# mrafidashti/neuradar

Measured on NVIDIA B200. Metric: train_step_rays_per_sec, higher is better.
Workload: dtype f32

## Files before the change

### neuradar_b200/csrc/field_fused.cu

```cuda
#include <algorithm>
#include <cstdlib>

#include <cuda.h>
#include <cuda_bf16.h>

#include "actor_grid.cuh"
#include "hash_bwd_plan.cuh"
#include "tc_common.cuh"

namespace nrb {

using namespace tc;

struct FusedParams {
  const float* w[5];
  const float* b[5];
  const float* beta;
  float beta_min;
};

__device__ constexpr int kLK[5] = {32, 32, 48, 32, 32};
__device__ constexpr int kLN[5] = {32, 48, 32, 32, 32};
__device__ constexpr int kLOut[5] = {32, 33, 32, 32, 32};

// ... 20 lines not shown
                   smem_u32(dst_smem)),
               "l"(src_gmem), "r"(bytes), "r"(smem_u32(mbar))
               : "memory");
}

__device__ __forceinline__ void mma_bf16_ss(uint32_t d_tmem, uint64_t a_desc, uint64_t b_desc, uint32_t idesc, bool acc) {
  asm volatile(
      "{\n\t"
      ".reg .pred p;\n\t"
      "setp.ne.b32 p, %4, 0;\n\t"
      "tcgen05.mma.cta_group::1.kind::f16 [%0], %1, %2, %3, p;\n\t"
      "}\n" ::"r"(d_tmem),
      "l"(a_desc), "l"(b_desc), "r"(idesc), "r"(static_cast<uint32_t>(acc))
      : "memory");
}

__device__ __forceinline__ void mma_bf16_ts(uint32_t d_tmem, uint32_t a_tmem, uint64_t b_desc, uint32_t idesc, bool acc) {
  asm volatile(
      "{\n\t"
      ".reg .pred p;\n\t"
      "setp.ne.b32 p, %4, 0;\n\t"
      "tcgen05.mma.cta_group::1.kind::f16 [%0], [%1], %2, %3, p;\n\t"
      "}\n" ::"r"(d_tmem),
      "r"(a_tmem), "l"(b_desc), "r"(idesc), "r"(static_cast<uint32_t>(acc))
      : "memory");
}

__device__ __forceinline__ uint32_t idesc_bf16(int m, int n, int a_mn_major, int b_mn_major) {
  return (1u << 4) | (1u << 7) | (1u << 10) | (static_cast<uint32_t>(a_mn_major) << 15) |
         (static_cast<uint32_t>(b_mn_major) << 16) | (static_cast<uint32_t>(n >> 3) << 17) |
         (static_cast<uint32_t>(m >> 4) << 24);
}

constexpr int kFGroups = 3;
constexpr int kFThreads = kFGroups * kRows;
constexpr int kFCols = 144;
constexpr int kFAcc = 0, kFAHi = 48, kFALo = 96;

__host__ __device__ constexpr int ff_w_floats(int l) { return l == 0 ? 32 * 32 : l == 1 ? 48 * 32 : l == 2 ? 32 * 48 : 32 * 32; }
__host__ __device__ constexpr int ff_w_hi(int l) {
  int o = 0;
  for (int i = 0; i < l; ++i) o += 2 * ff_w_floats(i) * 4;
  return o;
}
__host__ __device__ constexpr int ff_w_lo(int l) { return ff_w_hi(l) + ff_w_floats(l) * 4; }

struct FusedFwdSmem {
  static constexpr int bias = ff_w_hi(5);
  static constexpr int bounce = bias + 5 * 48 * 4;
  static constexpr int mbar = bounce + (kFThreads / 32) * 4096;
  static constexpr int tmem = mbar + 8 * kFGroups;
  static constexpr int total = tmem + 16;
};

struct FusedFwdArgs {
  const float* xyz;
  const float* std;
  const float* x;
  const float* sh;
  int samples_per_ray;
  int64_t M;
  float* feature;
  float* sdf;
  float* alpha;
  uint4* ximg;
  uint32_t* masks;
  int64_t ld;
  ActorGridsDev ag;
  ActorSamplesDev as;
};

template <int F, bool kActors>
__global__ void __launch_bounds__(kFThreads, 1) field_fused_fwd_kernel(const __grid_constant__ FusedParams prm,
                                                                       const __grid_constant__ GridDev grid,
                                                                       const __grid_constant__ FusedFwdArgs a) {
  extern __shared__ __align__(128) char smem[];
  const int t = threadIdx.x, lane = t & 31, r = t & (kRows - 1);
  const int uwarp = uniform_warp_idx();
  const int g = uwarp >> 2;
  float* s_bias = reinterpret_cast<float*>(smem + FusedFwdSmem::bias);
  uint64_t* mbar = reinterpret_cast<uint64_t*>(smem + FusedFwdSmem::mbar) + g;
  uint32_t* tmem_slot = reinterpret_cast<uint32_t*>(smem + FusedFwdSmem::tmem);
  char* bounce = smem + FusedFwdSmem::bounce + uwarp * 4096;

  for (int l = 0; l < 5; ++l) {
    stage_weight_split(prm.w[l], kLOut[l], kLN[l], kLK[l], smem + ff_w_hi(l), smem + ff_w_lo(l));
    for (int j = t; j < 48; j += kFThreads) s_bias[l * 48 + j] = (j < kLOut[l] && prm.b[l] != nullptr) ? __ldg(prm.b[l] + j) : 0.0f;
  }
  if (uwarp == 0) tmem_alloc<512>(tmem_slot);
  if (t == 0)
    for (int i = 0; i < kFGroups; ++i) mbar_init(reinterpret_cast<uint64_t*>(smem + FusedFwdSmem::mbar) + i, 1);
  fence_async_smem();
  fence_before_sync();
  __syncthreads();
  fence_after_sync();
  const uint32_t tg = *tmem_slot + static_cast<uint32_t>(g * kFCols);
  const uint32_t lane_base = tg + (static_cast<uint32_t>((uwarp & 3) * 32) << 16);
  const float beta = fabsf(__ldg(prm.beta)) + prm.beta_min;
  const bool train = a.ximg != nullptr;
  uint32_t phase = 0;

  auto run_layer = [&](int l) {
    fence_before_sync();
    group_barrier(g);
    if ((uwarp & 3) == 0) {
      if (elect_one()) {
        fence_after_sync();
        issue_gemm_ts(tg + kFAcc, kLN[l], tg + kFAHi, tg + kFALo, smem_u32(smem + ff_w_hi(l)), smem_u32(smem + ff_w_lo(l)),
                      kLK[l], kLK[l]);
        mma_commit(mbar);
      }
      __syncwarp();
    }
    mbar_wait(mbar, phase);
    phase ^= 1;
    fence_after_sync();
  };

  const int64_t tiles = (a.M + kRows - 1) / kRows;
  for (int64_t tile = blockIdx.x + static_cast<int64_t>(g) * gridDim.x; tile < tiles;
       tile += static_cast<int64_t>(kFGroups) * gridDim.x) {
    const int64_t row = tile * kRows + r;
    const bool ok = row < a.M;
    const int64_t rr = ok ? row : (a.M - 1);
    float v[32];
    int agid = -1;
    if constexpr (kActors) agid = __ldg(a.as.grid_id + rr);
    if (kActors && agid >= 0) {
      float o16[16];
      actor_gather16(a.ag, agid, __ldg(a.as.pos + 3 * rr), __ldg(a.as.pos + 3 * rr + 1), __ldg(a.as.pos + 3 * rr + 2),
                     __ldg(a.as.std + rr), o16);
#pragma unroll
      for (int j = 0; j < 16; ++j) {
        v[j] = o16[j];
        v[16 + j] = 0.0f;
      }
    } else if constexpr (F > 0) {
      const float px = __ldg(a.xyz + 3 * rr), py = __ldg(a.xyz + 3 * rr + 1), pz = __ldg(a.xyz + 3 * rr + 2);
      const float sd = a.std != nullptr ? __ldg(a.std + rr) : 0.0f;
      const uint32_t hmask = (1u << grid.log2_size) - 1u;
      constexpr int kBatch = 8 / F;
#pragma unroll
      for (int l0 = 0; l0 < 32 / F; l0 += kBatch) {
        Cell c[kBatch];
        float f[kBatch][8][F];
#pragma unroll
        for (int i = 0; i < kBatch; ++i) {
          c[i] = locate_cell(px, py, pz, grid.scalings[l0 + i], hmask);
          const float* base = grid.table + (static_cast<size_t>(l0 + i) << grid.log2_size) * F;
#pragma unroll
          for (int k = 0; k < 8; ++k) load_row<F>(base, c[i].row[k], f[i][k]);
        }
#pragma unroll
        for (int i = 0; i < kBatch; ++i) {
          const float ax = c[i].ox, bx = 1.0f - c[i].ox, ay = c[i].oy, by = 1.0f - c[i].oy, az = c[i].oz, bz = 1.0f - c[i].oz;
          const float w = a.std != nullptr ? level_weight(grid.scalings[l0 + i], sd) : 1.0f;
#pragma unroll
          for (int j = 0; j < F; ++j) {
            const float f03 = f[i][0][j] * ax + f[i][3][j] * bx;
            const float f12 = f[i][1][j] * ax + f[i][2][j] * bx;
            const float f56 = f[i][5][j] * ax + f[i][6][j] * bx;
            const float f47 = f[i][4][j] * ax + f[i][7][j] * bx;
            const float f0312 = f03 * ay + f12 * by;
            const float f4756 = f47 * ay + f56 * by;
            v[(l0 + i) * F + j] = (f0312 * az + f4756 * bz) * w;
          }
        }
      }
    } else {
      float4 pf[8];
      warp_load_rows_coalesced(a.x, tile * kRows + (uwarp & 3) * 32, a.M, lane, pf);
      warp_bounce_to_rows(bounce, lane, pf, v);
    }
    tmem_store_row_split<32>(tg, uwarp, kFAHi, kFALo, 0, v);
    if (train) {
#pragma unroll
      for (int q = 0; q < 4; ++q) {
        uint32_t h[4], m[4];
#pragma unroll
        for (int c = 0; c < 4; ++c) split_bf16_pair(v[8 * q + 2 * c], v[8 * q + 2 * c + 1], h[c], m[c]);
        uint4* dst = a.ximg + tile * 1024 + q * 128 + r;
        dst[0] = make_uint4(h[0], h[1], h[2], h[3]);
        dst[512] = make_uint4(m[0], m[1], m[2], m[3]);
      }
    }
    auto relu_mask = [&](const float* bias) {
      uint32_t m = 0;
#pragma unroll
      for (int j = 0; j < 32; ++j) {
        v[j] = fmaxf(v[j] + bias[j], 0.0f);
        m |= (v[j] > 0.0f ? 1u : 0u) << j;
      }
      return m;
    };
    run_layer(0);
    tmem_load_row<32>(tg + kFAcc, uwarp, 0, v);
    const uint32_t m_h1 = relu_mask(s_bias);
    tmem_store_row_split<32>(tg, uwarp, kFAHi, kFALo, 0, v);
    run_layer(1);
    float sdf_v;
    float emb[32];
    {
      float geo[48];
      tmem_load_row<48>(tg + kFAcc, uwarp, 0, geo);
      sdf_v = geo[0] + s_bias[48];
#pragma unroll
      for (int j = 0; j < 32; ++j) emb[j] = geo[1 + j] + s_bias[48 + 1 + j];
    }
    tmem_store_row_split<32>(tg, uwarp, kFAHi, kFALo, 0, emb);
    {
      float shv[16];
      if (kActors && agid >= 0) {
        sh16_of_direction(__ldg(a.as.dirs + 3 * rr), __ldg(a.as.dirs + 3 * rr + 1), __ldg(a.as.dirs + 3 * rr + 2), shv);
      } else {
        const float4* shp = reinterpret_cast<const float4*>(a.sh + (rr / a.samples_per_ray) * 16);
#pragma unroll
        for (int c = 0; c < 4; ++c) {
          const float4 q4 = __ldg(shp + c);
          shv[4 * c] = q4.x;
          shv[4 * c + 1] = q4.y;
          shv[4 * c + 2] = q4.z;
          shv[4 * c + 3] = q4.w;
        }
      }
      tmem_store_row_split<16>(tg, uwarp, kFAHi, kFALo, 32, shv);
    }
    run_layer(2);
    tmem_load_row<32>(tg + kFAcc, uwarp, 0, v);
    const uint32_t m_g1 = relu_mask(s_bias + 2 * 48);
    tmem_store_row_split<32>(tg, uwarp, kFAHi, kFALo, 0, v);
    run_layer(3);
    tmem_load_row<32>(tg + kFAcc, uwarp, 0, v);
    const uint32_t m_g2 = relu_mask(s_bias + 3 * 48);
    tmem_store_row_split<32>(tg, uwarp, kFAHi, kFALo, 0, v);
    if (train && ok) {
      a.masks[row] = m_h1;
      a.masks[a.ld + row] = m_g1;
      a.masks[2 * a.ld + row] = m_g2;
    }
    run_layer(4);
    tmem_load_row<32>(tg + kFAcc, uwarp, 0, v);
#pragma unroll
    for (int j = 0; j < 32; ++j) v[j] = emb[j] + (v[j] + s_bias[4 * 48 + j]);
    warp_store_rows_coalesced(a.feature, tile * kRows + (uwarp & 3) * 32, a.M, bounce, lane, v);
    if (ok) {
      a.sdf[row] = sdf_v;
      a.alpha[row] = 1.0f / (1.0f + expf(sdf_v * beta));
    }
  }
  fence_before_sync();
  __syncthreads();
  if (uwarp == 0) tmem_free<512>(*tmem_slot);
}

constexpr int kBGroups = 2;
constexpr int kBWorkers = kBGroups * kRows;
constexpr int kBIssuers = 1;
constexpr int kBThreads = kBWorkers + kBIssuers * 32;
constexpr int kBCols = 112;
constexpr int kBAcc = 0, kBAHi = 32, kBAMid = 56, kBDHi = 80, kBDMid = 96;
__device__ constexpr int kDwCol[5] = {224, 224, 368, 296, 296};
__device__ constexpr int kDwLane[5] = {0, 16, 0, 0, 16};
constexpr int kSdfCol = 368, kSdfLane = 16;

struct FusedBwdSmem {
  static constexpr int d_hi = 0, d_mid = 8192;
  static constexpr int d_sdf = 16384;
  static constexpr int d_bytes = 18432;
  static constexpr int h1 = d_bytes;
  static constexpr int emb = h1 + 18432;
  static constexpr int g1 = emb + 26624;
  static constexpr int g2x = g1 + 18432;
  static constexpr int group_bytes = g2x + 18432;
  static constexpr int w = kBGroups * group_bytes;
  static constexpr int w_bytes = 4 * 4096 + 6144;
  static constexpr int w1row0 = w + w_bytes;
// ... 562 lines not shown
              "nrb_field_fused_fwd: pass either a grid (+ xyz) to gather from or the hash features x");
  int F = 0;
  GridDev gd{};
  if (grid != nullptr) {
    if (int rc = check_grid(grid)) return rc;
    NRB_REQUIRE(xyz != nullptr, NRB_ERR_BAD_ARG, "nrb_field_fused_fwd: xyz is null");
    F = grid->features_per_level;
    NRB_REQUIRE((F == 2 || F == 4) && grid->num_levels * F == 32, NRB_ERR_UNSUPPORTED,
                "nrb_field_fused_fwd: the fused gather needs num_levels * features_per_level == 32 with 2 or 4 features");
    gd = to_dev(grid);
  } else {
    NRB_REQUIRE(aligned16(x), NRB_ERR_ALIGNMENT, "nrb_field_fused_fwd: x must be 16-byte aligned");
  }
  NRB_REQUIRE(aligned16(sh) && aligned16(feature), NRB_ERR_ALIGNMENT, "nrb_field_fused_fwd: sh and feature must be 16-byte aligned");
  if (M == 0) return NRB_OK;
  FusedFwdArgs a{};
  a.xyz = xyz, a.std = std, a.x = x, a.sh = sh, a.samples_per_ray = samples_per_ray, a.M = M;
  a.feature = feature, a.sdf = sdf, a.alpha = alpha;
  if (saved != nullptr && saved->ximg != nullptr) {
    NRB_REQUIRE(saved->masks != nullptr && saved->ld >= M && saved->ld % tc::kRows == 0 && aligned16(saved->ximg),
                NRB_ERR_BAD_ARG, "nrb_field_fused_fwd: saved.masks / saved.ld (nrb_field_saved_ld(M)) / alignment");
    a.ximg = static_cast<uint4*>(saved->ximg), a.masks = saved->masks, a.ld = saved->ld;
  }
  const bool actors = actor_grids != nullptr;
  if (actors) {
    if (int rc = check_actor_grids("nrb_field_fused_fwd", actor_grids)) return rc;
    NRB_REQUIRE(grid != nullptr && actor_samples && actor_samples->grid_id && actor_samples->pos && actor_samples->std &&
                    actor_samples->dirs,
                NRB_ERR_BAD_ARG, "nrb_field_fused_fwd: actors need the gather mode and all per-sample actor arrays");
    a.ag = to_dev(actor_grids);
    a.as = ActorSamplesDev{actor_samples->grid_id, actor_samples->pos, actor_samples->std, actor_samples->dirs};
  }
  const int64_t tiles = (M + tc::kRows - 1) / tc::kRows;
  const unsigned nblk = static_cast<unsigned>(std::min<int64_t>((tiles + kFGroups - 1) / kFGroups, sm_count()));
  auto s = static_cast<cudaStream_t>(stream);
#define NRB_FUSED_FWD(FF, AA)                                                                                                  \
  {                                                                                                                            \
    cudaError_t e = ensure_dynamic_smem(reinterpret_cast<const void*>(field_fused_fwd_kernel<FF, AA>), FusedFwdSmem::total); \
    NRB_REQUIRE(e == cudaSuccess, static_cast<int>(e), "nrb_field_fused_fwd: cudaFuncSetAttribute: %s", cudaGetErrorString(e));  \
    field_fused_fwd_kernel<FF, AA><<<nblk, kFThreads, FusedFwdSmem::total, s>>>(fused_params(p), gd, a);                       \
  }
  if (F == 2 && actors) NRB_FUSED_FWD(2, true) else if (F == 4 && actors) NRB_FUSED_FWD(4, true)
  else if (F == 2) NRB_FUSED_FWD(2, false) else if (F == 4) NRB_FUSED_FWD(4, false) else NRB_FUSED_FWD(0, false)
#undef NRB_FUSED_FWD
  return finish_launch("nrb_field_fused_fwd");
}

extern "C" int nrb_field_fused_bwd(const nrb_field_mlp_t* p, const nrb_field_fused_bwd_in_t* in,
                                   const nrb_field_fused_bwd_out_t* out, int32_t samples_per_ray, int64_t M,
                                   nrb_stream_t stream) {
  NRB_REQUIRE(p && in && out && M >= 0 && samples_per_ray > 0, NRB_ERR_BAD_ARG, "nrb_field_fused_bwd: null pointer or bad size");
  NRB_REQUIRE(in->saved.ximg && in->saved.masks && in->sh && in->sdf && in->alpha, NRB_ERR_BAD_ARG,
              "nrb_field_fused_bwd: a required input is null");
  NRB_REQUIRE((in->dfeature != nullptr) != (in->dfeat_ray != nullptr && in->weights != nullptr), NRB_ERR_BAD_ARG,
              "nrb_field_fused_bwd: pass either dfeature [M,32] or dfeat_ray [rays,32] with weights [M]");
  NRB_REQUIRE(in->saved.ld >= M && in->saved.ld % tc::kRows == 0, NRB_ERR_BAD_ARG,
              "nrb_field_fused_bwd: saved.ld must be nrb_field_saved_ld(M)");
  for (int l = 0; l < 5; ++l) NRB_REQUIRE(p->weights[l] != nullptr, NRB_ERR_BAD_ARG, "nrb_field_fused_bwd: weights[%d] is null", l);
  NRB_REQUIRE(p->beta != nullptr, NRB_ERR_BAD_ARG, "nrb_field_fused_bwd: beta is null");
  NRB_REQUIRE(aligned16(in->saved.ximg) && aligned16(in->sh) && (in->dfeature == nullptr || aligned16(in->dfeature)) &&
                  (in->dfeat_ray == nullptr || aligned16(in->dfeat_ray)) && (out->dximg == nullptr || aligned16(out->dximg)),
              NRB_ERR_ALIGNMENT, "nrb_field_fused_bwd: arrays must be 16-byte aligned");
  if (M == 0) return NRB_OK;
  FusedBwdArgs a{};
  a.ximg = static_cast<const uint4*>(in->saved.ximg), a.masks = in->saved.masks, a.ld = in->saved.ld;
  a.sh = in->sh, a.sdf = in->sdf, a.alpha = in->alpha;
  a.dfeature = in->dfeature, a.dfeat_ray = in->dfeat_ray, a.weights = in->weights, a.dsdf = in->dsdf, a.dalpha = in->dalpha;
// ... 29 lines not shown
```

### neuradar_b200/csrc/hash_bwd_plan.cuh

```cuda
#pragma once

#include <algorithm>

#include "common.cuh"

namespace nrb {

struct GridDev {
  const float* table;
  float scalings[NRB_MAX_LEVELS];
  int num_levels;
  int log2_size;
};

inline GridDev to_dev(const nrb_grid_t* g) {
  GridDev d;
  d.table = g->table;
  for (int i = 0; i < NRB_MAX_LEVELS; ++i) d.scalings[i] = g->scalings[i];
  d.num_levels = g->num_levels;
  d.log2_size = g->log2_hashmap_size;
  return d;
}

struct BwdPlan {
  float* scratch;
  int64_t offset[NRB_MAX_LEVELS];
  int64_t stride[NRB_MAX_LEVELS];
  int copies[NRB_MAX_LEVELS];
  int r1[NRB_MAX_LEVELS];
};

template <int F>
__device__ __forceinline__ void scatter_row(float* __restrict__ base, uint32_t row, const float (&v)[F]) {
  float* p = base + static_cast<size_t>(row) * F;
  if constexpr (F == 1) {
    atomicAdd(p, v[0]);
  } else if constexpr (F == 2) {
    atomicAdd(reinterpret_cast<float2*>(p), make_float2(v[0], v[1]));
  } else {
    atomicAdd(reinterpret_cast<float4*>(p), make_float4(v[0], v[1], v[2], v[3]));
  }
}

template <int F>
__device__ __forceinline__ void scatter_x_pair(float* __restrict__ base, uint32_t row_f, uint32_t row_c,
                                               const float (&vf)[F], const float (&vc)[F]) {
  if (row_c == row_f) {
    float t[F];
#pragma unroll
    for (int j = 0; j < F; ++j) t[j] = vf[j] + vc[j];
    scatter_row<F>(base, row_f, t);
    return;
  }
  if constexpr (F <= 2) {
    if (row_c == (row_f ^ 1u)) {
      const bool f_low = (row_f & 1u) == 0;
      float* p = base + static_cast<size_t>(row_f & ~1u) * F;
      if constexpr (F == 1) {
        atomicAdd(reinterpret_cast<float2*>(p), f_low ? make_float2(vf[0], vc[0]) : make_float2(vc[0], vf[0]));
      } else {
        atomicAdd(reinterpret_cast<float4*>(p), f_low ? make_float4(vf[0], vf[1], vc[0], vc[1])
                                                      : make_float4(vc[0], vc[1], vf[0], vf[1]));
      }
      return;
    }
  }
  scatter_row<F>(base, row_f, vf);
  scatter_row<F>(base, row_c, vc);
}

template <int F>
__device__ __forceinline__ void scatter_rows8(float* __restrict__ base, const uint32_t (&row)[8], const float (&v)[8][F]) {
  scatter_x_pair<F>(base, row[3], row[0], v[3], v[0]);
  scatter_x_pair<F>(base, row[2], row[1], v[2], v[1]);
  scatter_x_pair<F>(base, row[7], row[4], v[7], v[4]);
  scatter_x_pair<F>(base, row[6], row[5], v[6], v[5]);
}

template <int F>
__device__ __forceinline__ void scatter_corners(const BwdPlan& plan, int l, int log2_size, int xf, int yf, int zf, int xc,
                                                int yc, int zc, const uint32_t (&hashed_rows)[8], const float (&v)[8][F],
                                                float* __restrict__ dtable, unsigned spread) {
  const int copies = plan.copies[l];
  if (copies > 1) {
    const int R1 = plan.r1[l];
    if (xf >= 0 && yf >= 0 && zf >= 0 && xc < R1 && yc < R1 && zc < R1) {
      float* rep = plan.scratch + plan.offset[l] + static_cast<size_t>(spread % static_cast<unsigned>(copies)) * plan.stride[l];
      const int cx[8] = {xc, xc, xf, xf, xc, xc, xf, xf};
      const int cy[8] = {yc, yf, yf, yc, yc, yf, yf, yc};
      const int cz[8] = {zc, zc, zc, zc, zf, zf, zf, zf};
      uint32_t rows[8];
#pragma unroll
      for (int k = 0; k < 8; ++k) rows[k] = static_cast<uint32_t>((cz[k] * R1 + cy[k]) * R1 + cx[k]);
      scatter_rows8<F>(rep, rows, v);
      return;
    }
  }
  scatter_rows8<F>(dtable + (static_cast<size_t>(l) << log2_size) * F, hashed_rows, v);
}

constexpr int kMergeMaxRuns = 26;

template <int F>
__device__ __forceinline__ void merge_runs_and_scatter(const BwdPlan& plan, int l, int log2_size, float px, float py,
                                                       float pz, float scal, const Cell& c, float (&v)[8][F], bool valid,
                                                       int lane, float* __restrict__ dtable, unsigned spread) {
  const float sx = mul(px, scal), sy = mul(py, scal), sz = mul(pz, scal);
  const int xf = static_cast<int>(floorf(sx)), yf = static_cast<int>(floorf(sy)), zf = static_cast<int>(floorf(sz));
  const int xc = static_cast<int>(ceilf(sx)), yc = static_cast<int>(ceilf(sy)), zc = static_cast<int>(ceilf(sz));
  const int ceq = (xc == xf ? 1 : 0) | (yc == yf ? 2 : 0) | (zc == zf ? 4 : 0) | (valid ? 8 : 0);
  const int pxf = __shfl_up_sync(kFull, xf, 1), pyf = __shfl_up_sync(kFull, yf, 1), pzf = __shfl_up_sync(kFull, zf, 1);
  const int pce = __shfl_up_sync(kFull, ceq, 1);
  const bool head = lane == 0 || pxf != xf || pyf != yf || pzf != zf || pce != ceq;
  const unsigned heads = __ballot_sync(kFull, head);
  bool issue = valid;
  if (__popc(heads) <= kMergeMaxRuns) {
    const unsigned above = heads & ~((2u << lane) - 1u);
    const int next_head = above != 0 ? __ffs(above) - 1 : 32;
#pragma unroll
    for (int d = 1; d < 32; d <<= 1) {
      const bool take = lane + d < next_head;
      if (!__any_sync(kFull, take)) break;
#pragma unroll
      for (int k = 0; k < 8; ++k)
#pragma unroll
        for (int j = 0; j < F; ++j) {
          const float t = __shfl_down_sync(kFull, v[k][j], d);
          if (take) v[k][j] += t;
        }
    }
    issue = valid && head;
// ... 53 lines not shown
```

### neuradar_b200/csrc/proposal_fused.cu

```cuda
#include "actor_grid.cuh"
#include "common.cuh"
#include "hash_bwd_plan.cuh"

namespace nrb {

constexpr int kPropWarps = 4;
constexpr int kMaxChunks = NRB_MAX_SAMPLES / 32;

struct PropGrid {
  const float* table;
  float scalings[NRB_MAX_LEVELS];
  const float* decoder;
  int num_levels;
  int log2_size;
  const int32_t* agid;
  const float* apos;
  const float* astd;
  ActorGridsDev ag;
  float* adtables[NRB_MAX_ACTORS];
};

template <int F, bool kSave>
__global__ void __launch_bounds__(kPropWarps * 32) proposal_fwd_kernel(
    const __grid_constant__ PropGrid g, const float* __restrict__ origins, const float* __restrict__ directions,
// ... 49 lines not shown
      } else {
        for (int l = 0; l < g.num_levels; ++l) {
          const float scal = g.scalings[l];
          const Cell c = locate_cell(q.x, q.y, q.z, scal, mask);
          float v[F];
          interpolate<F>(g.table + (static_cast<size_t>(l) << g.log2_size) * F, c, v);
          const float lw = level_weight(scal, q.std);
#pragma unroll
          for (int j = 0; j < F; ++j) {
            const float f = v[j] * lw;
            pre = fmaf(f, s_dec[l * F + j], pre);
            if constexpr (kSave) saved_feats[(n * S + i) * LF + l * F + j] = f;
          }
        }
      }
      dens = expf(pre);
      if constexpr (kSave) saved_pre[n * S + i] = pre;
      if (density != nullptr) density[n * S + i] = dens;
      dd = mul(sub(end, start), dens);
    }
    const float incl = warp_inclusive_sum(dd, lane);
    float excl = __shfl_up_sync(kFull, incl, 1);
    if (lane == 0) excl = 0.0f;
    const float alpha = 1.0f - expf(-dd);
    const float trans = expf(-(carry + excl));
    if (ok) weights[n * S + i] = nan_to_num(alpha * trans);
    carry += __shfl_sync(kFull, incl, 31);
  }
}

template <int F, int kChunks>
__global__ void __launch_bounds__(kPropWarps * 32) proposal_bwd_kernel(
    const __grid_constant__ PropGrid g, const __grid_constant__ BwdPlan plan, const float* __restrict__ origins, const float* __restrict__ directions,
    const float* __restrict__ pixel_area, float scale, nrb_intervals_t iv, int64_t N,
    const float* __restrict__ saved_feats, const float* __restrict__ saved_pre, const float* __restrict__ dweights,
    const float* __restrict__ ddensity, float* __restrict__ dtable, float* __restrict__ ddecoder) {
  __shared__ float s_ddec[NRB_MAX_LEVELS * 4];
  __shared__ float s_dec[NRB_MAX_LEVELS * 4];
  const int lane = threadIdx.x & 31;
  const int S = iv.num_samples;
  const int LF = g.num_levels * F;
  if (threadIdx.x < NRB_MAX_LEVELS * 4) {
    s_ddec[threadIdx.x] = 0.0f;
    s_dec[threadIdx.x] = threadIdx.x < LF ? g.decoder[threadIdx.x] : 0.0f;
  }
  __syncthreads();
  const int64_t n = static_cast<int64_t>(blockIdx.x) * kPropWarps + (threadIdx.x >> 5);
  if (n < N) {
    const float ox = origins[3 * n], oy = origins[3 * n + 1], oz = origins[3 * n + 2];
    const float dx = directions[3 * n], dy = directions[3 * n + 1], dz = directions[3 * n + 2];
    const float pa = pixel_area[n];
    const float* st = iv.starts + n * iv.row_stride;
    const float* en = iv.ends + n * iv.row_stride;
    const uint32_t mask = (1u << g.log2_size) - 1u;
    float delta[kChunks], dd[kChunks], trans[kChunks], pre[kChunks], gdens[kChunks];
    float carry = 0.0f;
#pragma unroll
    for (int c = 0; c < kChunks; ++c) {
      if (c * 32 < S) {
        const int i = c * 32 + lane;
        const bool ok = i < S;
        pre[c] = ok ? saved_pre[n * S + i] : 0.0f;
        delta[c] = ok ? sub(en[i], st[i]) : 0.0f;
        dd[c] = ok ? mul(delta[c], expf(pre[c])) : 0.0f;
        const float incl = warp_inclusive_sum(dd[c], lane);
        float excl = __shfl_up_sync(kFull, incl, 1);
        if (lane == 0) excl = 0.0f;
        trans[c] = expf(-(carry + excl));
        carry += __shfl_sync(kFull, incl, 31);
      }
    }
    float suffix = 0.0f;
#pragma unroll
    for (int c = kChunks - 1; c >= 0; --c) {
      if (c * 32 < S) {
        const int i = c * 32 + lane;
        const bool ok = i < S;
        const float e = expf(-dd[c]);
        const float w = (1.0f - e) * trans[c];
        float gwt = (ok && dweights != nullptr) ? dweights[n * S + i] : 0.0f;
        if (isnan(w) || isinf(w)) gwt = 0.0f;
        const float gw = ok ? gwt * w : 0.0f;
        float incl = gw;
#pragma unroll
        for (int o = 1; o < 32; o <<= 1) {
          const float v = __shfl_down_sync(kFull, incl, o);
          if (lane + o < 32) incl += v;
        }
        float excl = __shfl_down_sync(kFull, incl, 1);
      if (lane == 31) excl = 0.0f;
      const float later = suffix + excl;
        gdens[c] = ok ? (gwt * trans[c] * e - later) * delta[c] : 0.0f;
        if (ok && ddensity != nullptr) gdens[c] += ddensity[n * S + i];
        suffix += __shfl_sync(kFull, incl, 0);
      }
    }
    const unsigned spread = static_cast<unsigned>(blockIdx.x * kPropWarps + (threadIdx.x >> 5));
#pragma unroll
    for (int c = 0; c < kChunks; ++c) {
      if (c * 32 < S) {
        const int i = c * 32 + lane;
        const bool act = i < S;
        const int ic = act ? i : (S - 1);
        const float gpre = act ? gdens[c] * expf(fminf(fmaxf(pre[c], -15.0f), 15.0f)) : 0.0f;
        const Gaussian q = sample_gaussian(ox, oy, oz, dx, dy, dz, pa, st[ic], en[ic], scale);
        const float* sf = saved_feats + (n * S + ic) * LF;
        const int agid = g.agid != nullptr ? g.agid[n * S + ic] : -1;
        if (act && agid >= 0) {
          const float ax = g.apos[3 * (n * S + ic)], ay = g.apos[3 * (n * S + ic) + 1], az = g.apos[3 * (n * S + ic) + 2];
          const float asd = g.astd[n * S + ic];
          const uint32_t amask = (1u << g.ag.log2_size) - 1u;
#pragma unroll
          for (int l = 0; l < kActorLevels; ++l) {
            const float scal = g.ag.scalings[l];
            const Cell cell = locate_cell(ax, ay, az, scal, amask);
            const float lw = level_weight(scal, asd);
            float gr[F];
#pragma unroll
            for (int j = 0; j < F; ++j) gr[j] = gpre * s_dec[l * F + j] * lw;
            float w8[8];
            corner_weights(cell, w8);
            float* dt = g.adtables[agid] + (static_cast<size_t>(l) << g.ag.log2_size) * F;
#pragma unroll
            for (int k = 0; k < 8; ++k) {
              float v[F];
#pragma unroll
              for (int j = 0; j < F; ++j) v[j] = gr[j] * w8[k];
              scatter_row<F>(dt, cell.row[k], v);
            }
          }
        }
        const bool act_static = act && agid < 0;
#pragma unroll 1
        for (int l = 0; l < g.num_levels; ++l) {
          const float scal = g.scalings[l];
          const Cell cell = locate_cell(q.x, q.y, q.z, scal, mask);
          const float lw = level_weight(scal, q.std);
          float gr[F];
#pragma unroll
          for (int j = 0; j < F; ++j) {
            const float dd_lj = warp_sum(gpre * sf[l * F + j]);
            if (lane == 0) atomicAdd(&s_ddec[l * F + j], dd_lj);
            gr[j] = gpre * s_dec[l * F + j] * lw;
          }
          float w8[8];
          corner_weights(cell, w8);
          float v[8][F];
#pragma unroll
          for (int k = 0; k < 8; ++k)
#pragma unroll
            for (int j = 0; j < F; ++j) v[k][j] = w8[k] * gr[j];
          merge_runs_and_scatter<F>(plan, l, g.log2_size, q.x, q.y, q.z, scal, cell, v, act_static, lane, dtable, spread);
        }
      }
    }
  }
  __syncthreads();
  if (threadIdx.x < LF && ddecoder != nullptr) atomicAdd(ddecoder + threadIdx.x, s_ddec[threadIdx.x]);
}

static PropGrid make_prop_grid(const nrb_grid_t* grid, const float* decoder, const nrb_actor_grids_t* agrids = nullptr,
                               const nrb_actor_samples_t* asamples = nullptr, float* const* adtables = nullptr) {
  PropGrid out{};
  if (agrids != nullptr) {
    out.ag = to_dev(agrids);
    out.agid = asamples->grid_id, out.apos = asamples->pos, out.astd = asamples->std;
    for (int i = 0; i < agrids->num_grids; ++i) out.adtables[i] = adtables != nullptr ? adtables[i] : nullptr;
  }
  out.table = grid->table;
  for (int i = 0; i < NRB_MAX_LEVELS; ++i) out.scalings[i] = grid->scalings[i];
  out.decoder = decoder;
  out.num_levels = grid->num_levels;
  out.log2_size = grid->log2_hashmap_size;
  return out;
}

static int check_proposal(const char* who, const nrb_rays_t* rays, const nrb_grid_t* grid, const float* decoder_w,
                          float scale, const nrb_intervals_t* iv) {
  if (int rc = check_rays(rays)) return rc;
  if (int rc = check_grid(grid)) return rc;
  if (int rc = check_intervals(who, iv)) return rc;
  NRB_REQUIRE(decoder_w != nullptr, NRB_ERR_BAD_ARG, "%s: null pointer", who);
  NRB_REQUIRE(scale > 0.f, NRB_ERR_BAD_ARG, "%s: static_scale must be positive", who);
  return NRB_OK;
}

}
// ... 24 lines not shown
  if (N == 0) return NRB_OK;
  const PropGrid g = make_prop_grid(grid, decoder_w, actor_grids, actor_samples);
  const unsigned blocks = blocks_for(N, kPropWarps);
  auto s = static_cast<cudaStream_t>(stream);
  const bool save = saved_feats != nullptr;
#define NRB_LAUNCH(F, SAVE)                                                                                          \
  proposal_fwd_kernel<F, SAVE><<<blocks, kPropWarps * 32, 0, s>>>(g, rays->origins, rays->directions,               \
                                                                  rays->pixel_area, static_scale, *iv, N,           \
                                                                  density, weights, saved_feats, saved_pre)
  switch (grid->features_per_level) {
    case 1: if (save) NRB_LAUNCH(1, true); else NRB_LAUNCH(1, false); break;
    case 2: if (save) NRB_LAUNCH(2, true); else NRB_LAUNCH(2, false); break;
    default: if (save) NRB_LAUNCH(4, true); else NRB_LAUNCH(4, false); break;
  }
#undef NRB_LAUNCH
  return finish_launch("nrb_proposal_fwd");
}

extern "C" int nrb_proposal_bwd(const nrb_rays_t* rays, const nrb_grid_t* grid, const float* decoder_w,
                                float static_scale, const nrb_intervals_t* iv, const float* saved_feats,
                                const float* saved_pre, const float* dweights, const float* ddensity, float* dtable,
                                float* ddecoder_w, void* workspace, int64_t workspace_bytes,
                                const nrb_actor_grids_t* actor_grids, const nrb_actor_samples_t* actor_samples,
                                float* const* actor_dtables, nrb_stream_t stream) {
  if (int rc = check_proposal("nrb_proposal_bwd", rays, grid, decoder_w, static_scale, iv)) return rc;
  if (int rc = check_prop_actors("nrb_proposal_bwd", grid, actor_grids, actor_samples)) return rc;
  NRB_REQUIRE(actor_grids == nullptr || actor_dtables != nullptr, NRB_ERR_BAD_ARG, "nrb_proposal_bwd: actor gradient tables missing");
  NRB_REQUIRE(saved_feats && saved_pre && dtable, NRB_ERR_BAD_ARG, "nrb_proposal_bwd: null pointer");
  NRB_REQUIRE(dweights || ddensity, NRB_ERR_BAD_ARG, "nrb_proposal_bwd: no upstream gradient");
  NRB_REQUIRE(aligned16(dtable), NRB_ERR_ALIGNMENT, "nrb_proposal_bwd: dtable must be 16-byte aligned");
  const int64_t N = rays->num_rays;
  if (N == 0) return NRB_OK;
  const PropGrid g = make_prop_grid(grid, decoder_w, actor_grids, actor_samples, actor_dtables);
  const unsigned blocks = blocks_for(N, kPropWarps);
  auto s = static_cast<cudaStream_t>(stream);
  BwdPlan plan;
  int64_t vertices = 0;
  if (int rc = prepare_bwd_plan(grid, N * iv->num_samples, workspace, workspace_bytes, s, &plan, &vertices)) return rc;
#define NRB_LAUNCH_C(F, CH)                                                                                        \
  proposal_bwd_kernel<F, CH><<<blocks, kPropWarps * 32, 0, s>>>(g, plan, rays->origins, rays->directions,          \
                                                                rays->pixel_area, static_scale, *iv, N, saved_feats, \
                                                                saved_pre, dweights, ddensity, dtable, ddecoder_w)
#define NRB_LAUNCH(F)                                   \
  if (iv->num_samples <= 64) {                          \
    NRB_LAUNCH_C(F, 2);                                 \
  } else if (iv->num_samples <= 128) {                  \
    NRB_LAUNCH_C(F, 4);                                 \
  } else {                                              \
    NRB_LAUNCH_C(F, kMaxChunks);                        \
  }
  switch (grid->features_per_level) {
    case 1: NRB_LAUNCH(1); break;
    case 2: NRB_LAUNCH(2); break;
    default: NRB_LAUNCH(4); break;
  }
#undef NRB_LAUNCH
#undef NRB_LAUNCH_C
  launch_fold(grid, plan, dtable, vertices, s);
  return finish_launch("nrb_proposal_bwd");
}
```

Before: 15.07 million.

## Warp-specialize fused field forward into gather producers and MLP consumers

Splits the forward kernel's warps into two dedicated gather groups that compute hash-grid or input features into a ring of shared-memory stages, and three MLP groups that consume those stages and run the tcgen05 layers. Full/empty mbarriers pass stages between the two roles, and setmaxnreg moves registers from the MLP warps to the gather warps. The aim is to overlap the latency-bound hash gathers with tensor-core MLP work instead of running them back to back in each group. The embedding is now parked in the stage buffer rather than held in registers. The cost is more shared memory, extra synchronisation, and a risk of register spills under the new caps.

New measurement: 14.78 million, median of 6. 0.981x the previous value.

```diff
diff --git a/neuradar_b200/csrc/field_fused.cu b/neuradar_b200/csrc/field_fused.cu
--- a/neuradar_b200/csrc/field_fused.cu
+++ b/neuradar_b200/csrc/field_fused.cu
@@ -76,10 +76,14 @@
          (static_cast<uint32_t>(m >> 4) << 24);
 }
 
-constexpr int kFGroups = 3;
-constexpr int kFThreads = kFGroups * kRows;
+constexpr int kFSlots = 3;
+constexpr int kFGather = 2;
+constexpr int kFStages = 6;
+constexpr int kFThreads = (kFSlots + kFGather) * kRows;
 constexpr int kFCols = 144;
 constexpr int kFAcc = 0, kFAHi = 48, kFALo = 96;
+constexpr int kFRegsMlp = 88, kFRegsGather = 104;
+static_assert(kFStages % kFSlots == 0 && kFStages % kFGather == 0, "a stage must have one producer and one consumer");
 
 __host__ __device__ constexpr int ff_w_floats(int l) { return l == 0 ? 32 * 32 : l == 1 ? 48 * 32 : l == 2 ? 32 * 48 : 32 * 32; }
 __host__ __device__ constexpr int ff_w_hi(int l) {
@@ -92,10 +96,13 @@
 struct FusedFwdSmem {
   static constexpr int bias = ff_w_hi(5);
   static constexpr int bounce = bias + 5 * 48 * 4;
-  static constexpr int mbar = bounce + (kFThreads / 32) * 4096;
-  static constexpr int tmem = mbar + 8 * kFGroups;
+  static constexpr int stage = bounce + (kFThreads / 32) * 4096;
+  static constexpr int stage_floats = 32 * kRows;
+  static constexpr int mbar = stage + kFStages * stage_floats * 4;
+  static constexpr int tmem = mbar + 8 * (kFSlots + 2 * kFStages);
   static constexpr int total = tmem + 16;
 };
+static_assert(FusedFwdSmem::total <= 227 * 1024, "forward shared memory");
 
 struct FusedFwdArgs {
   const float* xyz;
@@ -114,6 +121,76 @@
   ActorSamplesDev as;
 };
 
+template <int F, bool kActors, typename Sink>
+__device__ __forceinline__ void field_input_row(const GridDev& grid, const FusedFwdArgs& a, int64_t tile, int64_t rr, int wq,
+                                                int lane, char* bounce, Sink&& sink) {
+  int agid = -1;
+  if constexpr (kActors) agid = __ldg(a.as.grid_id + rr);
+  if (kActors && agid >= 0) {
+    float o16[16];
+    actor_gather16(a.ag, agid, __ldg(a.as.pos + 3 * rr), __ldg(a.as.pos + 3 * rr + 1), __ldg(a.as.pos + 3 * rr + 2),
+                   __ldg(a.as.std + rr), o16);
+#pragma unroll
+    for (int q = 0; q < 4; ++q) {
+      float v8[8];
+#pragma unroll
+      for (int j = 0; j < 8; ++j) v8[j] = q < 2 ? o16[8 * q + j] : 0.0f;
+      sink(q, v8);
+    }
+  } else if constexpr (F > 0) {
+    const float px = __ldg(a.xyz + 3 * rr), py = __ldg(a.xyz + 3 * rr + 1), pz = __ldg(a.xyz + 3 * rr + 2);
+    const float sd = a.std != nullptr ? __ldg(a.std + rr) : 0.0f;
+    const uint32_t hmask = (1u << grid.log2_size) - 1u;
+    constexpr int kBatch = 8 / F;
+#pragma unroll 1
+    for (int l0 = 0; l0 < 32 / F; l0 += kBatch) {
+      float v[8];
+      Cell c[kBatch];
+      float f[kBatch][8][F];
+#pragma unroll
+      for (int i = 0; i < kBatch; ++i) {
+        c[i] = locate_cell(px, py, pz, grid.scalings[l0 + i], hmask);
+        const float* base = grid.table + (static_cast<size_t>(l0 + i) << grid.log2_size) * F;
+#pragma unroll
+        for (int k = 0; k < 8; ++k) load_row<F>(base, c[i].row[k], f[i][k]);
+      }
+#pragma unroll
+      for (int i = 0; i < kBatch; ++i) {
+        const float ax = c[i].ox, bx = 1.0f - c[i].ox, ay = c[i].oy, by = 1.0f - c[i].oy, az = c[i].oz, bz = 1.0f - c[i].oz;
+        const float w = a.std != nullptr ? level_weight(grid.scalings[l0 + i], sd) : 1.0f;
+#pragma unroll
+        for (int j = 0; j < F; ++j) {
+          const float f03 = f[i][0][j] * ax + f[i][3][j] * bx;
+          const float f12 = f[i][1][j] * ax + f[i][2][j] * bx;
+          const float f56 = f[i][5][j] * ax + f[i][6][j] * bx;
+          const float f47 = f[i][4][j] * ax + f[i][7][j] * bx;
+          const float f0312 = f03 * ay + f12 * by;
+          const float f4756 = f47 * ay + f56 * by;
+          v[i * F + j] = (f0312 * az + f4756 * bz) * w;
+        }
+      }
+      sink(l0 * F / 8, v);
+    }
+  } else {
+    float4 pf[8];
+    float v[32];
+    warp_load_rows_coalesced(a.x, tile * kRows + wq * 32, a.M, lane, pf);
+    warp_bounce_to_rows(bounce, lane, pf, v);
+#pragma unroll
+    for (int q = 0; q < 4; ++q) {
+      float v8[8];
+#pragma unroll
+      for (int j = 0; j < 8; ++j) v8[j] = v[8 * q + j];
+      sink(q, v8);
+    }
+  }
+}
+
+template <int kRegs>
+__device__ __forceinline__ void setmaxnreg_inc() { asm volatile("setmaxnreg.inc.sync.aligned.u32 %0;" ::"n"(kRegs)); }
+template <int kRegs>
+__device__ __forceinline__ void setmaxnreg_dec() { asm volatile("setmaxnreg.dec.sync.aligned.u32 %0;" ::"n"(kRegs)); }
+
 template <int F, bool kActors>
 __global__ void __launch_bounds__(kFThreads, 1) field_fused_fwd_kernel(const __grid_constant__ FusedParams prm,
                                                                        const __grid_constant__ GridDev grid,
@@ -123,7 +200,10 @@
   const int uwarp = uniform_warp_idx();
   const int g = uwarp >> 2;
   float* s_bias = reinterpret_cast<float*>(smem + FusedFwdSmem::bias);
-  uint64_t* mbar = reinterpret_cast<uint64_t*>(smem + FusedFwdSmem::mbar) + g;
+  uint64_t* mb_mma = reinterpret_cast<uint64_t*>(smem + FusedFwdSmem::mbar);
+  uint64_t* mb_full = mb_mma + kFSlots;
+  uint64_t* mb_empty = mb_full + kFStages;
+  float* stages = reinterpret_cast<float*>(smem + FusedFwdSmem::stage);
   uint32_t* tmem_slot = reinterpret_cast<uint32_t*>(smem + FusedFwdSmem::tmem);
   char* bounce = smem + FusedFwdSmem::bounce + uwarp * 4096;
 
@@ -132,16 +212,50 @@
     for (int j = t; j < 48; j += kFThreads) s_bias[l * 48 + j] = (j < kLOut[l] && prm.b[l] != nullptr) ? __ldg(prm.b[l] + j) : 0.0f;
   }
   if (uwarp == 0) tmem_alloc<512>(tmem_slot);
-  if (t == 0)
-    for (int i = 0; i < kFGroups; ++i) mbar_init(reinterpret_cast<uint64_t*>(smem + FusedFwdSmem::mbar) + i, 1);
+  if (t == 0) {
+    for (int i = 0; i < kFSlots; ++i) mbar_init(mb_mma + i, 1);
+    for (int i = 0; i < 2 * kFStages; ++i) mbar_init(mb_full + i, kRows);
+  }
   fence_async_smem();
   fence_before_sync();
   __syncthreads();
   fence_after_sync();
+  const bool train = a.ximg != nullptr;
+  const int64_t tiles = (a.M + kRows - 1) / kRows;
+  const int64_t mine = static_cast<int64_t>(blockIdx.x) < tiles ? (tiles - 1 - blockIdx.x) / gridDim.x + 1 : 0;
+
+  if (g >= kFSlots) {
+    setmaxnreg_inc<kFRegsGather>();
+    for (int64_t k = g - kFSlots; k < mine; k += kFGather) {
+      const int64_t tile = blockIdx.x + k * gridDim.x;
+      const int64_t row = tile * kRows + r;
+      const int64_t rr = row < a.M ? row : (a.M - 1);
+      const int s = static_cast<int>(k % kFStages);
+      mbar_wait(mb_empty + s, static_cast<uint32_t>((k / kFStages) & 1) ^ 1u);
+      float* st = stages + s * FusedFwdSmem::stage_floats;
+      field_input_row<F, kActors>(grid, a, tile, rr, uwarp & 3, lane, bounce, [&](int q, const float (&v)[8]) {
+#pragma unroll
+        for (int j = 0; j < 8; ++j) st[(8 * q + j) * kRows + r] = v[j];
+        if (train) {
+          uint32_t h[4], m[4];
+#pragma unroll
+          for (int c = 0; c < 4; ++c) split_bf16_pair(v[2 * c], v[2 * c + 1], h[c], m[c]);
+          uint4* dst = a.ximg + tile * 1024 + q * 128 + r;
+          dst[0] = make_uint4(h[0], h[1], h[2], h[3]);
+          dst[512] = make_uint4(m[0], m[1], m[2], m[3]);
+        }
+      });
+      mbar_arrive(mb_full + s);
+    }
+    fence_before_sync();
+    __syncthreads();
+    return;
+  }
+
+  setmaxnreg_dec<kFRegsMlp>();
+  uint64_t* mbar = mb_mma + g;
   const uint32_t tg = *tmem_slot + static_cast<uint32_t>(g * kFCols);
-  const uint32_t lane_base = tg + (static_cast<uint32_t>((uwarp & 3) * 32) << 16);
   const float beta = fabsf(__ldg(prm.beta)) + prm.beta_min;
-  const bool train = a.ximg != nullptr;
   uint32_t phase = 0;
 
   auto run_layer = [&](int l) {
@@ -161,73 +275,20 @@
     fence_after_sync();
   };
 
-  const int64_t tiles = (a.M + kRows - 1) / kRows;
-  for (int64_t tile = blockIdx.x + static_cast<int64_t>(g) * gridDim.x; tile < tiles;
-       tile += static_cast<int64_t>(kFGroups) * gridDim.x) {
+  for (int64_t k = g; k < mine; k += kFSlots) {
+    const int64_t tile = blockIdx.x + k * gridDim.x;
     const int64_t row = tile * kRows + r;
     const bool ok = row < a.M;
     const int64_t rr = ok ? row : (a.M - 1);
-    float v[32];
     int agid = -1;
     if constexpr (kActors) agid = __ldg(a.as.grid_id + rr);
-    if (kActors && agid >= 0) {
-      float o16[16];
-      actor_gather16(a.ag, agid, __ldg(a.as.pos + 3 * rr), __ldg(a.as.pos + 3 * rr + 1), __ldg(a.as.pos + 3 * rr + 2),
-                     __ldg(a.as.std + rr), o16);
-#pragma unroll
-      for (int j = 0; j < 16; ++j) {
-        v[j] = o16[j];
-        v[16 + j] = 0.0f;
-      }
-    } else if constexpr (F > 0) {
-      const float px = __ldg(a.xyz + 3 * rr), py = __ldg(a.xyz + 3 * rr + 1), pz = __ldg(a.xyz + 3 * rr + 2);
-      const float sd = a.std != nullptr ? __ldg(a.std + rr) : 0.0f;
-      const uint32_t hmask = (1u << grid.log2_size) - 1u;
-      constexpr int kBatch = 8 / F;
-#pragma unroll
-      for (int l0 = 0; l0 < 32 / F; l0 += kBatch) {
-        Cell c[kBatch];
-        float f[kBatch][8][F];
-#pragma unroll
-        for (int i = 0; i < kBatch; ++i) {
-          c[i] = locate_cell(px, py, pz, grid.scalings[l0 + i], hmask);
-          const float* base = grid.table + (static_cast<size_t>(l0 + i) << grid.log2_size) * F;
-#pragma unroll
-          for (int k = 0; k < 8; ++k) load_row<F>(base, c[i].row[k], f[i][k]);
-        }
-#pragma unroll
-        for (int i = 0; i < kBatch; ++i) {
-          const float ax = c[i].ox, bx = 1.0f - c[i].ox, ay = c[i].oy, by = 1.0f - c[i].oy, az = c[i].oz, bz = 1.0f - c[i].oz;
-          const float w = a.std != nullptr ? level_weight(grid.scalings[l0 + i], sd) : 1.0f;
-#pragma unroll
-          for (int j = 0; j < F; ++j) {
-            const float f03 = f[i][0][j] * ax + f[i][3][j] * bx;
-            const float f12 = f[i][1][j] * ax + f[i][2][j] * bx;
-            const float f56 = f[i][5][j] * ax + f[i][6][j] * bx;
-            const float f47 = f[i][4][j] * ax + f[i][7][j] * bx;
-            const float f0312 = f03 * ay + f12 * by;
-            const float f4756 = f47 * ay + f56 * by;
-            v[(l0 + i) * F + j] = (f0312 * az + f4756 * bz) * w;
-          }
-        }
-      }
-    } else {
-      float4 pf[8];
-      warp_load_rows_coalesced(a.x, tile * kRows + (uwarp & 3) * 32, a.M, lane, pf);
-      warp_bounce_to_rows(bounce, lane, pf, v);
-    }
+    const int s = static_cast<int>(k % kFStages);
+    float* st = stages + s * FusedFwdSmem::stage_floats;
+    float v[32];
+    mbar_wait(mb_full + s, static_cast<uint32_t>((k / kFStages) & 1));
+#pragma unroll
+    for (int j = 0; j < 32; ++j) v[j] = st[j * kRows + r];
     tmem_store_row_split<32>(tg, uwarp, kFAHi, kFALo, 0, v);
-    if (train) {
-#pragma unroll
-      for (int q = 0; q < 4; ++q) {
-        uint32_t h[4], m[4];
-#pragma unroll
-        for (int c = 0; c < 4; ++c) split_bf16_pair(v[8 * q + 2 * c], v[8 * q + 2 * c + 1], h[c], m[c]);
-        uint4* dst = a.ximg + tile * 1024 + q * 128 + r;
-        dst[0] = make_uint4(h[0], h[1], h[2], h[3]);
-        dst[512] = make_uint4(m[0], m[1], m[2], m[3]);
-      }
-    }
     auto relu_mask = [&](const float* bias) {
       uint32_t m = 0;
 #pragma unroll
@@ -243,15 +304,16 @@
     tmem_store_row_split<32>(tg, uwarp, kFAHi, kFALo, 0, v);
     run_layer(1);
     float sdf_v;
-    float emb[32];
     {
-      float geo[48];
+      float geo[48], emb[32];
       tmem_load_row<48>(tg + kFAcc, uwarp, 0, geo);
       sdf_v = geo[0] + s_bias[48];
 #pragma unroll
       for (int j = 0; j < 32; ++j) emb[j] = geo[1 + j] + s_bias[48 + 1 + j];
-    }
-    tmem_store_row_split<32>(tg, uwarp, kFAHi, kFALo, 0, emb);
+#pragma unroll
+      for (int j = 0; j < 32; ++j) st[j * kRows + r] = emb[j];
+      tmem_store_row_split<32>(tg, uwarp, kFAHi, kFALo, 0, emb);
+    }
     {
       float shv[16];
       if (kActors && agid >= 0) {
@@ -285,7 +347,8 @@
     run_layer(4);
     tmem_load_row<32>(tg + kFAcc, uwarp, 0, v);
 #pragma unroll
-    for (int j = 0; j < 32; ++j) v[j] = emb[j] + (v[j] + s_bias[4 * 48 + j]);
+    for (int j = 0; j < 32; ++j) v[j] = st[j * kRows + r] + (v[j] + s_bias[4 * 48 + j]);
+    mbar_arrive(mb_empty + s);
     warp_store_rows_coalesced(a.feature, tile * kRows + (uwarp & 3) * 32, a.M, bounce, lane, v);
     if (ok) {
       a.sdf[row] = sdf_v;
@@ -914,7 +977,7 @@
     a.as = ActorSamplesDev{actor_samples->grid_id, actor_samples->pos, actor_samples->std, actor_samples->dirs};
   }
   const int64_t tiles = (M + tc::kRows - 1) / tc::kRows;
-  const unsigned nblk = static_cast<unsigned>(std::min<int64_t>((tiles + kFGroups - 1) / kFGroups, sm_count()));
+  const unsigned nblk = static_cast<unsigned>(std::min<int64_t>((tiles + kFSlots - 1) / kFSlots, sm_count()));
   auto s = static_cast<cudaStream_t>(stream);
 #define NRB_FUSED_FWD(FF, AA)                                                                                                  \
   {                                                                                                                            \
```

## Stage per-sample gradients in shared memory and pack sample work across warps

Applied to the files above, without the earlier changes.

The proposal backward kernel now runs in two phases. Phase one computes per-sample density gradients per ray into dynamic shared memory. Phase two flattens all samples in the block into dense 32-lane chunks split across warps, so idle lanes from sample counts that are not multiples of 32 are removed from the expensive hash-grid scatter. Separately, the F=1 scatter now merges corner pairs falling in the same aligned group of four rows into a single float4 atomic. The cost is extra shared memory, a block-wide barrier, and re-reading ray data per sample.

Result: faster. 15.09 million before, 15.67 million after (median of 6 runs) (+3.8%).

```diff
diff --git a/neuradar_b200/csrc/hash_bwd_plan.cuh b/neuradar_b200/csrc/hash_bwd_plan.cuh
--- a/neuradar_b200/csrc/hash_bwd_plan.cuh
+++ b/neuradar_b200/csrc/hash_bwd_plan.cuh
@@ -44,7 +44,7 @@
 
 template <int F>
 __device__ __forceinline__ void scatter_x_pair(float* __restrict__ base, uint32_t row_f, uint32_t row_c,
-                                               const float (&vf)[F], const float (&vc)[F]) {
+                                               const float (&vf)[F], const float (&vc)[F], bool quad) {
   if (row_c == row_f) {
     float t[F];
 #pragma unroll
@@ -52,16 +52,19 @@
     scatter_row<F>(base, row_f, t);
     return;
   }
-  if constexpr (F <= 2) {
+  if constexpr (F == 1) {
+    if (quad && (row_f ^ row_c) < 4u) {
+      const uint32_t sf = row_f & 3u, sc = row_c & 3u;
+      const float4 t = make_float4(sf == 0 ? vf[0] : (sc == 0 ? vc[0] : 0.0f), sf == 1 ? vf[0] : (sc == 1 ? vc[0] : 0.0f),
+                                   sf == 2 ? vf[0] : (sc == 2 ? vc[0] : 0.0f), sf == 3 ? vf[0] : (sc == 3 ? vc[0] : 0.0f));
+      atomicAdd(reinterpret_cast<float4*>(base) + (row_f >> 2), t);
+      return;
+    }
+  } else if constexpr (F == 2) {
     if (row_c == (row_f ^ 1u)) {
       const bool f_low = (row_f & 1u) == 0;
-      float* p = base + static_cast<size_t>(row_f & ~1u) * F;
-      if constexpr (F == 1) {
-        atomicAdd(reinterpret_cast<float2*>(p), f_low ? make_float2(vf[0], vc[0]) : make_float2(vc[0], vf[0]));
-      } else {
-        atomicAdd(reinterpret_cast<float4*>(p), f_low ? make_float4(vf[0], vf[1], vc[0], vc[1])
-                                                      : make_float4(vc[0], vc[1], vf[0], vf[1]));
-      }
+      atomicAdd(reinterpret_cast<float4*>(base) + (row_f >> 1), f_low ? make_float4(vf[0], vf[1], vc[0], vc[1])
+                                                                     : make_float4(vc[0], vc[1], vf[0], vf[1]));
       return;
     }
   }
@@ -70,11 +73,12 @@
 }
 
 template <int F>
-__device__ __forceinline__ void scatter_rows8(float* __restrict__ base, const uint32_t (&row)[8], const float (&v)[8][F]) {
-  scatter_x_pair<F>(base, row[3], row[0], v[3], v[0]);
-  scatter_x_pair<F>(base, row[2], row[1], v[2], v[1]);
-  scatter_x_pair<F>(base, row[7], row[4], v[7], v[4]);
-  scatter_x_pair<F>(base, row[6], row[5], v[6], v[5]);
+__device__ __forceinline__ void scatter_rows8(float* __restrict__ base, const uint32_t (&row)[8], const float (&v)[8][F],
+                                              bool quad) {
+  scatter_x_pair<F>(base, row[3], row[0], v[3], v[0], quad);
+  scatter_x_pair<F>(base, row[2], row[1], v[2], v[1], quad);
+  scatter_x_pair<F>(base, row[7], row[4], v[7], v[4], quad);
+  scatter_x_pair<F>(base, row[6], row[5], v[6], v[5], quad);
 }
 
 template <int F>
@@ -92,11 +96,11 @@
       uint32_t rows[8];
 #pragma unroll
       for (int k = 0; k < 8; ++k) rows[k] = static_cast<uint32_t>((cz[k] * R1 + cy[k]) * R1 + cx[k]);
-      scatter_rows8<F>(rep, rows, v);
+      scatter_rows8<F>(rep, rows, v, true);
       return;
     }
   }
-  scatter_rows8<F>(dtable + (static_cast<size_t>(l) << log2_size) * F, hashed_rows, v);
+  scatter_rows8<F>(dtable + (static_cast<size_t>(l) << log2_size) * F, hashed_rows, v, log2_size >= 2);
 }
 
 constexpr int kMergeMaxRuns = 26;
diff --git a/neuradar_b200/csrc/proposal_fused.cu b/neuradar_b200/csrc/proposal_fused.cu
--- a/neuradar_b200/csrc/proposal_fused.cu
+++ b/neuradar_b200/csrc/proposal_fused.cu
@@ -105,28 +105,28 @@
 template <int F, int kChunks>
 __global__ void __launch_bounds__(kPropWarps * 32) proposal_bwd_kernel(
     const __grid_constant__ PropGrid g, const __grid_constant__ BwdPlan plan, const float* __restrict__ origins, const float* __restrict__ directions,
-    const float* __restrict__ pixel_area, float scale, nrb_intervals_t iv, int64_t N,
+    const float* __restrict__ pixel_area, float scale, nrb_intervals_t iv, int64_t N, int rays_per_block,
     const float* __restrict__ saved_feats, const float* __restrict__ saved_pre, const float* __restrict__ dweights,
     const float* __restrict__ ddensity, float* __restrict__ dtable, float* __restrict__ ddecoder) {
+  extern __shared__ float s_gpre[];
   __shared__ float s_ddec[NRB_MAX_LEVELS * 4];
   __shared__ float s_dec[NRB_MAX_LEVELS * 4];
   const int lane = threadIdx.x & 31;
+  const int warp = threadIdx.x >> 5;
   const int S = iv.num_samples;
   const int LF = g.num_levels * F;
   if (threadIdx.x < NRB_MAX_LEVELS * 4) {
     s_ddec[threadIdx.x] = 0.0f;
     s_dec[threadIdx.x] = threadIdx.x < LF ? g.decoder[threadIdx.x] : 0.0f;
   }
-  __syncthreads();
-  const int64_t n = static_cast<int64_t>(blockIdx.x) * kPropWarps + (threadIdx.x >> 5);
-  if (n < N) {
-    const float ox = origins[3 * n], oy = origins[3 * n + 1], oz = origins[3 * n + 2];
-    const float dx = directions[3 * n], dy = directions[3 * n + 1], dz = directions[3 * n + 2];
-    const float pa = pixel_area[n];
+  const int64_t n0 = static_cast<int64_t>(blockIdx.x) * rays_per_block;
+  const int rays = static_cast<int>(min(static_cast<int64_t>(rays_per_block), N - n0));
+#pragma unroll 1
+  for (int r = warp; r < rays; r += kPropWarps) {
+    const int64_t n = n0 + r;
     const float* st = iv.starts + n * iv.row_stride;
     const float* en = iv.ends + n * iv.row_stride;
-    const uint32_t mask = (1u << g.log2_size) - 1u;
-    float delta[kChunks], dd[kChunks], trans[kChunks], pre[kChunks], gdens[kChunks];
+    float delta[kChunks], dd[kChunks], trans[kChunks], pre[kChunks];
     float carry = 0.0f;
 #pragma unroll
     for (int c = 0; c < kChunks; ++c) {
@@ -161,71 +161,84 @@
           if (lane + o < 32) incl += v;
         }
         float excl = __shfl_down_sync(kFull, incl, 1);
-      if (lane == 31) excl = 0.0f;
-      const float later = suffix + excl;
-        gdens[c] = ok ? (gwt * trans[c] * e - later) * delta[c] : 0.0f;
-        if (ok && ddensity != nullptr) gdens[c] += ddensity[n * S + i];
+        if (lane == 31) excl = 0.0f;
+        const float later = suffix + excl;
+        if (ok) {
+          float gdens = (gwt * trans[c] * e - later) * delta[c];
+          if (ddensity != nullptr) gdens += ddensity[n * S + i];
+          s_gpre[r * S + i] = gdens * expf(fminf(fmaxf(pre[c], -15.0f), 15.0f));
+        }
         suffix += __shfl_sync(kFull, incl, 0);
       }
     }
-    const unsigned spread = static_cast<unsigned>(blockIdx.x * kPropWarps + (threadIdx.x >> 5));
-#pragma unroll
-    for (int c = 0; c < kChunks; ++c) {
-      if (c * 32 < S) {
-        const int i = c * 32 + lane;
-        const bool act = i < S;
-        const int ic = act ? i : (S - 1);
-        const float gpre = act ? gdens[c] * expf(fminf(fmaxf(pre[c], -15.0f), 15.0f)) : 0.0f;
-        const Gaussian q = sample_gaussian(ox, oy, oz, dx, dy, dz, pa, st[ic], en[ic], scale);
-        const float* sf = saved_feats + (n * S + ic) * LF;
-        const int agid = g.agid != nullptr ? g.agid[n * S + ic] : -1;
-        if (act && agid >= 0) {
-          const float ax = g.apos[3 * (n * S + ic)], ay = g.apos[3 * (n * S + ic) + 1], az = g.apos[3 * (n * S + ic) + 2];
-          const float asd = g.astd[n * S + ic];
-          const uint32_t amask = (1u << g.ag.log2_size) - 1u;
-#pragma unroll
-          for (int l = 0; l < kActorLevels; ++l) {
-            const float scal = g.ag.scalings[l];
-            const Cell cell = locate_cell(ax, ay, az, scal, amask);
-            const float lw = level_weight(scal, asd);
-            float gr[F];
-#pragma unroll
-            for (int j = 0; j < F; ++j) gr[j] = gpre * s_dec[l * F + j] * lw;
-            float w8[8];
-            corner_weights(cell, w8);
-            float* dt = g.adtables[agid] + (static_cast<size_t>(l) << g.ag.log2_size) * F;
-#pragma unroll
-            for (int k = 0; k < 8; ++k) {
-              float v[F];
-#pragma unroll
-              for (int j = 0; j < F; ++j) v[j] = gr[j] * w8[k];
-              scatter_row<F>(dt, cell.row[k], v);
-            }
-          }
-        }
-        const bool act_static = act && agid < 0;
+  }
+  __syncthreads();
+  const int total = rays * S;
+  const int chunks = (total + 31) >> 5;
+  const int per_warp = (chunks + kPropWarps - 1) / kPropWarps;
+  const int c_end = min(chunks, (warp + 1) * per_warp);
+  const unsigned spread = static_cast<unsigned>(blockIdx.x * kPropWarps + warp);
+  const uint32_t mask = (1u << g.log2_size) - 1u;
 #pragma unroll 1
-        for (int l = 0; l < g.num_levels; ++l) {
-          const float scal = g.scalings[l];
-          const Cell cell = locate_cell(q.x, q.y, q.z, scal, mask);
-          const float lw = level_weight(scal, q.std);
-          float gr[F];
-#pragma unroll
-          for (int j = 0; j < F; ++j) {
-            const float dd_lj = warp_sum(gpre * sf[l * F + j]);
-            if (lane == 0) atomicAdd(&s_ddec[l * F + j], dd_lj);
-            gr[j] = gpre * s_dec[l * F + j] * lw;
-          }
-          float w8[8];
-          corner_weights(cell, w8);
-          float v[8][F];
-#pragma unroll
-          for (int k = 0; k < 8; ++k)
-#pragma unroll
-            for (int j = 0; j < F; ++j) v[k][j] = w8[k] * gr[j];
-          merge_runs_and_scatter<F>(plan, l, g.log2_size, q.x, q.y, q.z, scal, cell, v, act_static, lane, dtable, spread);
-        }
-      }
+  for (int c = warp * per_warp; c < c_end; ++c) {
+    const int k = c * 32 + lane;
+    const bool act = k < total;
+    const int kc = act ? k : total - 1;
+    const int r = kc / S;
+    const int i = kc - r * S;
+    const int64_t n = n0 + r;
+    const int64_t m = n0 * S + kc;
+    const float gpre = act ? s_gpre[kc] : 0.0f;
+    const Gaussian q = sample_gaussian(origins[3 * n], origins[3 * n + 1], origins[3 * n + 2], directions[3 * n],
+                                       directions[3 * n + 1], directions[3 * n + 2], pixel_area[n],
+                                       iv.starts[n * iv.row_stride + i], iv.ends[n * iv.row_stride + i], scale);
+    const float* sf = saved_feats + m * LF;
+    const int agid = g.agid != nullptr ? g.agid[m] : -1;
+    if (act && agid >= 0) {
+      const float ax = g.apos[3 * m], ay = g.apos[3 * m + 1], az = g.apos[3 * m + 2];
+      const float asd = g.astd[m];
+      const uint32_t amask = (1u << g.ag.log2_size) - 1u;
+#pragma unroll
+      for (int l = 0; l < kActorLevels; ++l) {
+        const float scal = g.ag.scalings[l];
+        const Cell cell = locate_cell(ax, ay, az, scal, amask);
+        const float lw = level_weight(scal, asd);
+        float gr[F];
+#pragma unroll
+        for (int j = 0; j < F; ++j) gr[j] = gpre * s_dec[l * F + j] * lw;
+        float w8[8];
+        corner_weights(cell, w8);
+        float* dt = g.adtables[agid] + (static_cast<size_t>(l) << g.ag.log2_size) * F;
+#pragma unroll
+        for (int k8 = 0; k8 < 8; ++k8) {
+          float v[F];
+#pragma unroll
+          for (int j = 0; j < F; ++j) v[j] = gr[j] * w8[k8];
+          scatter_row<F>(dt, cell.row[k8], v);
+        }
+      }
+    }
+    const bool act_static = act && agid < 0;
+#pragma unroll 1
+    for (int l = 0; l < g.num_levels; ++l) {
+      const float scal = g.scalings[l];
+      const Cell cell = locate_cell(q.x, q.y, q.z, scal, mask);
+      const float lw = level_weight(scal, q.std);
+      float gr[F];
+#pragma unroll
+      for (int j = 0; j < F; ++j) {
+        const float dd_lj = warp_sum(gpre * sf[l * F + j]);
+        if (lane == 0) atomicAdd(&s_ddec[l * F + j], dd_lj);
+        gr[j] = gpre * s_dec[l * F + j] * lw;
+      }
+      float w8[8];
+      corner_weights(cell, w8);
+      float v[8][F];
+#pragma unroll
+      for (int k8 = 0; k8 < 8; ++k8)
+#pragma unroll
+        for (int j = 0; j < F; ++j) v[k8][j] = w8[k8] * gr[j];
+      merge_runs_and_scatter<F>(plan, l, g.log2_size, q.x, q.y, q.z, scal, cell, v, act_static, lane, dtable, spread);
     }
   }
   __syncthreads();
@@ -316,15 +329,20 @@
   const int64_t N = rays->num_rays;
   if (N == 0) return NRB_OK;
   const PropGrid g = make_prop_grid(grid, decoder_w, actor_grids, actor_samples, actor_dtables);
-  const unsigned blocks = blocks_for(N, kPropWarps);
+  int rays_per_block = kPropWarps;
+  while (rays_per_block < 4 * kPropWarps && (rays_per_block * iv->num_samples) % (kPropWarps * 32) != 0) rays_per_block *= 2;
+  if ((rays_per_block * iv->num_samples) % (kPropWarps * 32) != 0) rays_per_block = kPropWarps;
+  const unsigned blocks = blocks_for(N, rays_per_block);
+  const size_t smem = static_cast<size_t>(rays_per_block) * iv->num_samples * sizeof(float);
   auto s = static_cast<cudaStream_t>(stream);
   BwdPlan plan;
   int64_t vertices = 0;
   if (int rc = prepare_bwd_plan(grid, N * iv->num_samples, workspace, workspace_bytes, s, &plan, &vertices)) return rc;
-#define NRB_LAUNCH_C(F, CH)                                                                                        \
-  proposal_bwd_kernel<F, CH><<<blocks, kPropWarps * 32, 0, s>>>(g, plan, rays->origins, rays->directions,          \
-                                                                rays->pixel_area, static_scale, *iv, N, saved_feats, \
-                                                                saved_pre, dweights, ddensity, dtable, ddecoder_w)
+#define NRB_LAUNCH_C(F, CH)                                                                                          \
+  proposal_bwd_kernel<F, CH><<<blocks, kPropWarps * 32, smem, s>>>(g, plan, rays->origins, rays->directions,         \
+                                                                   rays->pixel_area, static_scale, *iv, N,           \
+                                                                   rays_per_block, saved_feats, saved_pre, dweights, \
+                                                                   ddensity, dtable, ddecoder_w)
 #define NRB_LAUNCH(F)                                   \
   if (iv->num_samples <= 64) {                          \
     NRB_LAUNCH_C(F, 2);                                 \
```
